# YifYang993/CR-NeRF-PyTorch

Measured on AMD Instinct MI355X. Metric: rays/sec (64+128 samples, 8-layer W=256 MLP), higher is better.
Workload: dtype f32

## Files before the change

cr-nerf-pytorch_amd/csrc/mlp_core.h:

```cpp
#pragma once
#include <hip/hip_runtime.h>
#include "layout.h"

namespace crnerf {

typedef float f32x16 __attribute__((ext_vector_type(16)));
typedef float f32x4 __attribute__((ext_vector_type(4)));
typedef __attribute__((address_space(3))) char lds_char;
typedef __attribute__((address_space(3))) float lds_float;
typedef __attribute__((address_space(3))) uint32_t lds_uint;
typedef const __attribute__((address_space(1))) char gbl_char;

constexpr int RING_SLOTS = 6;
static_assert(RING_SLOTS >= 5, "ring too shallow for the read-ahead protocol");

constexpr int LDS_CONST0 = 0;
constexpr int LDS_CONST1 = CONST_BYTES;
constexpr int LDS_RING = 2 * CONST_BYTES;
constexpr int LDS_SCRATCH = LDS_RING + RING_SLOTS * STAGE_BYTES;

enum { T_PROLOGUE = 0, T_MMA, T_EPILOGUE, T_SIGMA, T_COMPOSITE, T_RAYLEVEL, T_TOTAL, T_X0, T_X1, T_X2, T_X3, T_X4, T_X5, T_X6, T_X7, T_REAL, T_COUNT };
#ifdef CRNERF_TIMING
static __device__ unsigned long long crnerf_timing[T_COUNT];
struct PhaseTimer {
  unsigned long long last, acc[T_COUNT], real0;
  bool on;
  __device__ __forceinline__ void start(bool on_) {
    on = on_;
    for (int i = 0; i < T_COUNT; ++i) acc[i] = 0;
    real0 = __builtin_amdgcn_s_memrealtime();
    last = __builtin_readcyclecounter();
  }
  __device__ __forceinline__ void tick(int phase) {
    __builtin_amdgcn_sched_barrier(0);
    const unsigned long long t = __builtin_readcyclecounter();
    __builtin_amdgcn_sched_barrier(0);
    acc[phase] += t - last;
    acc[T_TOTAL] += t - last;
    last = t;
  }
  __device__ __forceinline__ void flush() {
    acc[T_REAL] = __builtin_amdgcn_s_memrealtime() - real0;
    if (on)
      for (int i = 0; i < T_COUNT; ++i) crnerf_timing[i] = acc[i];
  }
};
#else
struct PhaseTimer {
  __device__ __forceinline__ void start(bool) {}
  __device__ __forceinline__ void tick(int) {}
  __device__ __forceinline__ void flush() {}
};
#endif

__device__ __forceinline__ void glds16(uint32_t lds_addr, const char* base, uint32_t voff, int imm) {
#ifdef CRNERF_GLDS_SALU_COPY
  uint64_t b;
  asm volatile("s_mov_b32 m0, %1\n\ts_mov_b64 %0, %3\n\tglobal_load_lds_dwordx4 %2, %0 offset:%4"
               : "=&s"(b) : "s"(lds_addr), "v"(voff), "s"(base), "n"(imm) : "memory");
#else
  asm volatile("s_mov_b32 m0, %0\n\ts_nop 0\n\tglobal_load_lds_dwordx4 %1, %2 offset:%3" ::"s"(lds_addr), "v"(voff), "s"(base), "n"(imm)
               : "memory");
#endif
}
__device__ __forceinline__ void glds16_more(const char* base, uint32_t voff, int imm) {
#ifdef CRNERF_GLDS_SALU_COPY
  uint64_t b;
  asm volatile("s_mov_b64 %0, %2\n\tglobal_load_lds_dwordx4 %1, %0 offset:%3" : "=&s"(b) : "v"(voff), "s"(base), "n"(imm) : "memory");
#else
  asm volatile("global_load_lds_dwordx4 %0, %1 offset:%2" ::"v"(voff), "s"(base), "n"(imm) : "memory");
#endif
}

template <int NT>
__device__ __forceinline__ void init_acc(f32x16 (&acc)[NT], const lds_float* bias, int h) {
#pragma unroll
  for (int t = 0; t < NT; ++t) {
#pragma unroll
    for (int q = 0; q < 4; ++q) {
      const f32x4 b = *(const __attribute__((address_space(3))) f32x4*)(bias + 32 * t + 8 * q + 4 * h);
      acc[t][4 * q + 0] = b[0];
      acc[t][4 * q + 1] = b[1];
      acc[t][4 * q + 2] = b[2];
      acc[t][4 * q + 3] = b[3];
    }
  }
}

template <int NT, int NDST>
__device__ __forceinline__ void store_act(const f32x16 (&acc)[NT], f32x16 (&act)[NDST], float floor_) {
#pragma unroll
  for (int t = 0; t < NT; ++t)
#pragma unroll
    for (int r = 0; r < 16; ++r) act[t][r] = fmaxf(acc[t][r], floor_);
}

__device__ __forceinline__ float softplus_ref(float x) {
  return x > 20.0f ? x : log1pf(expf(x));
}
__device__ __forceinline__ float sigmoid_ref(float x) { return 1.0f / (1.0f + expf(-x)); }

__device__ __forceinline__ void load_consts(lds_char* lds, const char* packed0, const char* packed1) {
  const int tid = threadIdx.x;
  for (int i = tid; i < CONST_BYTES / 16; i += blockDim.x) {
    const f32x4 a = *(const f32x4*)(packed0 + i * 16);
    const f32x4 b = *(const f32x4*)(packed1 + i * 16);
    *(__attribute__((address_space(3))) f32x4*)(lds + LDS_CONST0 + i * 16) = a;
    *(__attribute__((address_space(3))) f32x4*)(lds + LDS_CONST1 + i * 16) = b;
  }
  __syncthreads();
}

}
```

cr-nerf-pytorch_amd/csrc/mlp_core16.h:

```cpp
#pragma once
#include <hip/hip_runtime.h>
#include "layout.h"
#include "sincos_pow2.h"
#include "mlp_core.h"

namespace crnerf {

#define CRNERF_MFMA16(a, b, c) __builtin_amdgcn_mfma_f32_16x16x4f32((a), (b), (c), 0, 0, 0)

constexpr int V16_WAVES = 8;
constexpr int V16_PIECES = STAGE_FRAGS / V16_WAVES;
constexpr int V16_AHEAD = 4;

constexpr int U_XYZ = XYZ_PAD / 16;
constexpr int U_HID = W_HIDDEN / 16;
constexpr int U_DIR = DIR_PAD / 16;
constexpr int U_HALF = 128 / 16;

constexpr int TRUNK_STAGES = OFF_FIN / STAGE_FRAGS;
static_assert(OFF_FIN % STAGE_FRAGS == 0, "the trunk must be whole stages");
template <bool TRUNK0>
struct WeightPipe16T {
  static constexpr bool trunk0 = TRUNK0;
  lds_char* lds;
  const char* base[2];
  const char* pf_ptr;
  int pf_left, pf_pass, passes0, passes;
  int stages_per_pass = STAGES_PER_PASS;
  uint32_t pf_slot, rd_slot, rd_addr, lane16, wave2k, lds_ring;
  int stagger;

  __device__ __forceinline__ void issue_piece(int i) {
    const uint32_t dst = lds_ring + pf_slot * STAGE_BYTES;
    if (i == 0) glds16(dst, pf_ptr, lane16, 0);
    else glds16(dst, pf_ptr, lane16, FRAG_BYTES);
    if (i == V16_PIECES - 1) {
      pf_slot = (pf_slot + 1 == RING_SLOTS) ? 0u : pf_slot + 1;
      pf_ptr += STAGE_BYTES;
      if (--pf_left == 0) {
        pf_left = stages_per_pass;
        pf_pass = (pf_pass + 1 == passes) ? 0 : pf_pass + 1;
        pf_ptr = (pf_pass < passes0) ? base[0] : base[1];
        if (TRUNK0 && pf_pass < passes0) pf_left = TRUNK_STAGES;
      }
    }
  }

  __device__ __forceinline__ void start(lds_char* lds_, const char* stream0, const char* stream1, int passes0_, int passes_,
                                        int lane, int wave) {
    static_assert(V16_PIECES == 2, "issue_piece hard-codes the two instruction offsets");
    lds = lds_;
    lane16 = (uint32_t)lane * 16u;
    wave2k = (uint32_t)wave * (V16_PIECES * FRAG_BYTES);
    lds_ring = (uint32_t)(uintptr_t)lds_ + LDS_RING + wave2k;
    stagger = (wave >> 2) & 1;
    base[0] = stream0 + wave2k;
    base[1] = stream1 + wave2k;
    passes0 = passes0_;
    passes = passes_;
    pf_pass = 0;
    pf_left = (TRUNK0 && passes0 > 0) ? TRUNK_STAGES : stages_per_pass;
    pf_ptr = (passes0 > 0) ? base[0] : base[1];
    pf_slot = 0;
    rd_slot = 0;
    rd_addr = LDS_RING + lane16;
#pragma unroll
    for (int s = 0; s < RING_SLOTS - 1; ++s)
#pragma unroll
      for (int i = 0; i < V16_PIECES; ++i) issue_piece(i);
    asm volatile("s_waitcnt vmcnt(%0)" ::"n"(V16_PIECES * (RING_SLOTS - 3)) : "memory");
    __builtin_amdgcn_s_barrier();
  }

  __device__ __forceinline__ uint32_t next_addr() const {
    const uint32_t n = (rd_slot + 1 == RING_SLOTS) ? 0u : rd_slot + 1;
    return LDS_RING + n * STAGE_BYTES + lane16;
  }

  __device__ __forceinline__ void advance() {
    asm volatile("s_waitcnt vmcnt(%0)" ::"n"(V16_PIECES * (RING_SLOTS - 4)) : "memory");
    __builtin_amdgcn_s_barrier();
    rd_slot = (rd_slot + 1 == RING_SLOTS) ? 0u : rd_slot + 1;
    rd_addr = LDS_RING + rd_slot * STAGE_BYTES + lane16;
  }

  __device__ __forceinline__ f32x4 read_slot(int s) const {
    const uint32_t a = (s < STAGE_FRAGS) ? rd_addr + s * FRAG_BYTES : next_addr() + (s - STAGE_FRAGS) * FRAG_BYTES;
    return *(const __attribute__((address_space(3))) f32x4*)(lds + a);
  }

  __device__ __forceinline__ void prime(f32x4 (&q)[V16_AHEAD]) const {
#pragma unroll
    for (int i = 0; i < V16_AHEAD; ++i) q[i] = read_slot(i);
  }
};
typedef WeightPipe16T<false> WeightPipe16;

template <int NT>
__device__ __forceinline__ void init_acc16(f32x4 (&acc)[NT], const lds_float* bias, int g) {
#pragma unroll
  for (int T = 0; T < NT; ++T) acc[T] = *(const __attribute__((address_space(3))) f32x4*)(bias + 16 * T + 4 * g);
}

struct NoDeferred {
  static constexpr int pieces = 0;
  __device__ __forceinline__ void piece(int) const {}
};
template <class SAVE, int ND>
struct DeferredActs {
  static constexpr int pieces = ND;
  const SAVE& save;
  float* row;
  const f32x4 (&a)[16];
  __device__ __forceinline__ void piece(int T) const { save.piece(row, T, a[T]); }
};

template <int NT, int NGA, int NGB, int NA, int NB, class DEF = NoDeferred, class PIPE>
__device__ __forceinline__ void mma_layer16(PIPE& p, const f32x4 (&srcA)[NA], const f32x4 (&srcB)[NB], f32x4 (&acc)[NT],
                                            f32x4 (&q)[V16_AHEAD], const DEF& def = DEF()) {
  static_assert(NGA <= NA && NGB <= NB, "source too small");
  constexpr int NF = (NGA + NGB) * NT;
  static_assert(NF % STAGE_FRAGS == 0 && NT % 2 == 0, "layer must be whole stages");
  constexpr int STEPS = NF / 2;
  constexpr int STRIDE = DEF::pieces > 0 ? (STEPS / DEF::pieces >= 4 ? 4 : (STEPS / DEF::pieces >= 2 ? 2 : 1)) : 1;
  static_assert(DEF::pieces == 0 || STRIDE * DEF::pieces <= STEPS, "not enough steps to carry the deferred stores");
#pragma unroll
  for (int u = 0; u < NGA + NGB; ++u) {
#pragma unroll
    for (int T = 0; T < NT; T += 2) {
      const int f = u * NT + T;
      const int s = f % STAGE_FRAGS;
      if (s % 4 == 0 && ((s >> 2) & 1) == p.stagger) p.issue_piece(s >> 3);
      const f32x4 a0 = q[f % V16_AHEAD], a1 = q[(f + 1) % V16_AHEAD];
      q[f % V16_AHEAD] = p.read_slot(s + V16_AHEAD);
      q[(f + 1) % V16_AHEAD] = p.read_slot(s + 1 + V16_AHEAD);
#pragma unroll
      for (int r = 0; r < 4; ++r) {
        const float b = (u < NGA) ? srcA[u < NGA ? u : 0][r] : srcB[u < NGA ? 0 : u - NGA][r];
        acc[T] = CRNERF_MFMA16(a0[r], b, acc[T]);
        acc[T + 1] = CRNERF_MFMA16(a1[r], b, acc[T + 1]);
      }
      if (s == STAGE_FRAGS - 2) p.advance();
      if (DEF::pieces > 0) {
        const int step = f / 2;
        if (step % STRIDE == 0 && step / STRIDE < DEF::pieces) def.piece(step / STRIDE);
      }
    }
  }
}

template <int NT, bool RELU, int NDST>
__device__ __forceinline__ void store_act16(const f32x4 (&acc)[NT], f32x4 (&act)[NDST]) {
#pragma unroll
  for (int T = 0; T < NT; ++T)
#pragma unroll
    for (int r = 0; r < 4; ++r) act[T][r] = RELU ? fmaxf(acc[T][r], 0.0f) : acc[T][r];
}

struct NoSave {
  template <int NT>
  __device__ __forceinline__ void operator()(int, const f32x4 (&)[NT]) const {}
  template <int NT>
  __device__ __forceinline__ float* begin(int, const f32x4 (&)[NT]) const { return nullptr; }
  __device__ __forceinline__ void piece(float*, int, const f32x4&) const {}
};

struct DirRegs {
  f32x4 v[2];
  __device__ __forceinline__ void get(f32x4 (&o)[2]) const { o[0] = v[0]; o[1] = v[1]; }
};
struct DirLds {
  const lds_float* p;
  __device__ __forceinline__ void get(f32x4 (&o)[2]) const {
    o[0] = *(const __attribute__((address_space(3))) f32x4*)(p);
    o[1] = *(const __attribute__((address_space(3))) f32x4*)(p + 4);
  }
};

template <class DIR, class SAVE = NoSave, class PIPE>
__device__ __forceinline__ void mlp_tile16(PIPE& p, int model, const f32x4 (&pe)[6], const DIR& dir,
                                           f32x4 (&feat)[4], float& sigma, int g, f32x4 (&q)[V16_AHEAD], PhaseTimer& tm,
                                           const SAVE& save = SAVE()) {
  const lds_float* C = (const lds_float*)(p.lds + (model ? LDS_CONST1 : LDS_CONST0));
  f32x4 act[16], acc[16];
  tm.tick(T_PROLOGUE);

  typedef DeferredActs<SAVE, 16> Def16;
  init_acc16<16>(acc, C + C_BIAS, g);
  mma_layer16<16, U_XYZ, 0>(p, pe, pe, acc, q);
  tm.tick(T_MMA);
  store_act16<16, true>(acc, act);
  float* row = save.begin(0, act);
#pragma unroll 1
  for (int l = 1; l < 4; ++l) {
    init_acc16<16>(acc, C + C_BIAS + l * W_HIDDEN, g);
    tm.tick(T_EPILOGUE);
    mma_layer16<16, U_HID, 0>(p, act, act, acc, q, Def16{save, row, act});
    tm.tick(T_MMA);
    store_act16<16, true>(acc, act);
    row = save.begin(l, act);
  }
  init_acc16<16>(acc, C + C_BIAS + 4 * W_HIDDEN, g);
  tm.tick(T_EPILOGUE);
  mma_layer16<16, U_XYZ, U_HID>(p, pe, act, acc, q, Def16{save, row, act});
  tm.tick(T_MMA);
  store_act16<16, true>(acc, act);
  row = save.begin(4, act);
#pragma unroll 1
  for (int l = 5; l < 8; ++l) {
    init_acc16<16>(acc, C + C_BIAS + l * W_HIDDEN, g);
    tm.tick(T_EPILOGUE);
    mma_layer16<16, U_HID, 0>(p, act, act, acc, q, Def16{save, row, act});
    tm.tick(T_MMA);
    store_act16<16, true>(acc, act);
    row = save.begin(l, act);
  }
  {
    float s0 = 0.0f, s1 = 0.0f;
#pragma unroll
    for (int T = 0; T < 16; T += 2) {
      const f32x4 w0 = *(const __attribute__((address_space(3))) f32x4*)(C + C_WSIG + 16 * T + 4 * g);
      const f32x4 w1 = *(const __attribute__((address_space(3))) f32x4*)(C + C_WSIG + 16 * (T + 1) + 4 * g);
#pragma unroll
      for (int r = 0; r < 4; ++r) {
        s0 = fmaf(w0[r], act[T][r], s0);
        s1 = fmaf(w1[r], act[T + 1][r], s1);
      }
    }
    float s = s0 + s1;
    s += __shfl_xor(s, 16);
    s += __shfl_xor(s, 32);
    sigma = softplus_ref(s + C[C_BSIG]);
  }
  tm.tick(T_SIGMA);
  if (PIPE::trunk0 && model == 0) {
#pragma unroll
    for (int T = 0; T < 4; ++T) feat[T] = f32x4{0, 0, 0, 0};
    return;
  }
  init_acc16<16>(acc, C + C_BFIN, g);
  mma_layer16<16, U_HID, 0>(p, act, act, acc, q, Def16{save, row, act});
  tm.tick(T_MMA);
  store_act16<16, false>(acc, act);
  row = save.begin(8, act);
  {
    f32x4 acc8[8], dv[2];
    dir.get(dv);
    init_acc16<8>(acc8, C + C_BDIR, g);
    tm.tick(T_EPILOGUE);
    mma_layer16<8, U_HID, U_DIR>(p, act, dv, acc8, q, Def16{save, row, act});
    tm.tick(T_MMA);
    store_act16<8, true>(acc8, act);
    row = save.begin(9, act);
  }
  {
    f32x4 acc4[4];
    init_acc16<4>(acc4, C + C_BRGB, g);
    tm.tick(T_EPILOGUE);
    mma_layer16<4, U_HALF, 0>(p, act, act, acc4, q, DeferredActs<SAVE, 8>{save, row, act});
    tm.tick(T_MMA);
#pragma unroll
    for (int T = 0; T < 4; ++T)
#pragma unroll
      for (int r = 0; r < 4; ++r) feat[T][r] = sigmoid_ref(acc4[T][r]);
  }
  tm.tick(T_EPILOGUE);
}

template <int F, int NV>
__device__ __forceinline__ void posenc_regs16(float x, float y, float z, int g, f32x4 (&out)[NV]) {
  const Rev2Pi rx = to_rev2pi(x), ry = to_rev2pi(y), rz = to_rev2pi(z);
#pragma unroll
  for (int v = 0; v < NV; ++v)
#pragma unroll
    for (int pr = 0; pr < 2; ++pr) {
      const int a_lo = 8 * v + pr;
      const int a = a_lo + 2 * g;
      float e0, e1;
      if (a_lo + 6 < 3 * F) {
        const int f = a / 3, d = a - 3 * f;
        const Rev2Pi val = {d == 0 ? rx.p : (d == 1 ? ry.p : rz.p), d == 0 ? rx.e : (d == 1 ? ry.e : rz.e)};
        float s, c;
        sincos_rev2pi(val, f, s, c);
        e0 = s; e1 = c;
      } else {
        const bool trig = a < 3 * F;
        const int ac = trig ? a : 0;
        const int f = ac / 3, d = ac - 3 * f;
        const Rev2Pi val = {d == 0 ? rx.p : (d == 1 ? ry.p : rz.p), d == 0 ? rx.e : (d == 1 ? ry.e : rz.e)};
        float s, c;
        sincos_rev2pi(val, f, s, c);
        e0 = trig ? s : (a == 3 * F ? x : (a == 3 * F + 1 ? z : 0.0f));
        e1 = trig ? c : (a == 3 * F ? y : 0.0f);
      }
      out[v][2 * pr + 0] = e0;
      out[v][2 * pr + 1] = e1;
    }
}

}
```

cr-nerf-pytorch_amd/csrc/render_fused16.hip:

```cpp
#include <hip/hip_runtime.h>
#include "kernels.h"
#include "mlp_core16.h"
#include "mlp_train16.h"
#include "pair_ops.h"
#include "ray_ops.h"

namespace crnerf {

struct RenderParams16 {
  const char* packed0; const char* packed1;
  const float* rays; const float* view_dir; const float* z_coarse; const float* z_steps; const float* u; long u_stride;
  const float* noise_c; const float* noise_f; float noise_std; int use_disp;
  long R; int Nc, Ni, iters;
  unsigned int* sched;
  float* weights_c; float* feature_c; float* depth_c; float* weights_f; float* feature_f; float* depth_f; float* z_fine;
  unsigned long long rng_seed; long rng_ray_offset; int rng_flags; float perturb;
  float* z_coarse_out; float* noise_c_out; float* noise_f_out;
};

static __device__ unsigned int crnerf_sched16[SCHED_SLOTS][2];

struct NoHook {
  __device__ __forceinline__ NoSave saver(int, long, int, int, bool, int) const { return NoSave(); }
  __device__ __forceinline__ void raw(int, long, int, int, bool, int, const f32x4 (&)[4], float) const {}
};
struct TrainHook {
  float* acts[2];
  float* rawo[2];
  long R;
  __device__ __forceinline__ ActSaver saver(int pass, long r, int N, int n, bool ok, int g) const {
    return ActSaver{pass ? acts[1] : acts[0], R * N, r * N + n, ok, g};
  }
  __device__ __forceinline__ void raw(int pass, long r, int N, int n, bool ok, int g, const f32x4 (&feat)[4], float sigma) const {
    if (!ok) return;
    float* o = (pass ? rawo[1] : rawo[0]) + (r * N + n) * OUT_DIM;
#pragma unroll
    for (int T = 0; T < 4; ++T)
#pragma unroll
      for (int q = 0; q < 4; ++q) o[16 * T + 4 * g + q] = feat[T][q];
    if (g == 0) o[FEAT_DIM] = sigma;
  }
};

template <bool RNG, class HOOK, bool LEAN = false>
__device__ __forceinline__ void render_rays16_impl(const RenderParams16& a, const HOOK& hook) {
  extern __shared__ __attribute__((aligned(16))) char smem[];
  lds_char* lds = (lds_char*)smem;
  const int lane = threadIdx.x & 63;
  const int wave = __builtin_amdgcn_readfirstlane(threadIdx.x >> 6);
  const int p = lane & 15, g = lane >> 4;
  const int pair = wave >> 1, half = wave & 1;
  const int lane128 = half * 64 + lane;
  const int Nc = a.Nc, Ni = a.Ni, Nf = Nc + Ni;

  load_consts(lds, a.packed0, a.packed1);
  PairScratch scr;
  scr.bind(lds + LDS_SCRATCH + pair * PAIR_BYTES);
  lds_float* dirbuf = (lds_float*)(lds + LDS_SCRATCH + 4 * PAIR_BYTES) + wave * 32;

  const int steps_c = (Nc + 31) >> 5, steps_f = Ni > 0 ? (Nf + 31) >> 5 : 0;
  WeightPipe16T<LEAN> pipe;
  pipe.start(lds, a.packed0 + CONST_BYTES, a.packed1 + CONST_BYTES, steps_c, steps_c + steps_f, lane, wave);
  f32x4 q[V16_AHEAD];
  pipe.prime(q);
  PhaseTimer tm;
  tm.start(blockIdx.x == 0 && threadIdx.x == 0);

  __attribute__((address_space(3))) unsigned int* qslot =
      (__attribute__((address_space(3))) unsigned int*)(lds + LDS_SCRATCH + 4 * PAIR_BYTES + V16_WAVES * 32 * sizeof(float));
  const long quads = (a.R + 3) / 4;
  long quad = blockIdx.x;
#pragma unroll 1
  for (int it = 0; a.sched ? quad < quads : it < a.iters; ++it) {
    unsigned int nxt = 0;
    if (a.sched && threadIdx.x == 0) nxt = gridDim.x + atomicAdd(a.sched, 1u);
    const long rr = quad * 4 + pair;
    const bool ray_ok = rr < a.R;
    const long r = ray_ok ? rr : a.R - 1;
    const float* ray = a.rays + r * 8;
    const float ox = ray[0], oy = ray[1], oz = ray[2], dx = ray[3], dy = ray[4], dz = ray[5];
    const float near = ray[6], far = ray[7];
    {
      const float* vd = a.view_dir ? a.view_dir + r * 3 : ray + 3;
      f32x4 dv[2];
      posenc_regs16<DIR_FREQS, 2>(vd[0], vd[1], vd[2], g, dv);
      if (p == 0) {
        *(__attribute__((address_space(3))) f32x4*)(dirbuf + 8 * g) = dv[0];
        *(__attribute__((address_space(3))) f32x4*)(dirbuf + 8 * g + 4) = dv[1];
      }
    }
    const DirLds dirsrc{dirbuf + 8 * g};
    const RayRng rng{(uint32_t)(a.rng_seed & 0xffffffffu), (uint32_t)(a.rng_seed >> 32)};
    const long rng_ray = a.rng_ray_offset + r;
    for (int n = lane128; n < Nc; n += 128) {
      auto zlin = [&](int k) { return coarse_depth(near, far, a.z_steps ? a.z_steps[k] : linspace01(k, Nc), a.use_disp); };
      float zv;
      if (a.z_coarse) zv = a.z_coarse[r * Nc + n];
      else if (RNG && (a.rng_flags & 1)) {
        const float z0 = zlin(n);
        const float lower = n == 0 ? z0 : 0.5f * (zlin(n - 1) + z0);
        const float upper = n == Nc - 1 ? z0 : 0.5f * (z0 + zlin(n + 1));
        zv = lower + (upper - lower) * (a.perturb * rng.uniform(RNG_STREAM_JITTER, rng_ray, n));
      } else zv = zlin(n);
      scr.zc[n] = zv;
      if (RNG && a.z_coarse_out && ray_ok) a.z_coarse_out[r * Nc + n] = zv;
    }
    wg_barrier();

    const int npass = Ni > 0 ? 2 : 1;
#pragma unroll 1
    for (int pass = 0; pass < npass; ++pass) {
      const int N = pass ? Nf : Nc;
      const lds_float* zsrc = pass ? scr.zs : scr.zc;
      const float* noise_row = pass ? (a.noise_f ? a.noise_f + r * Nf : nullptr) : (a.noise_c ? a.noise_c + r * Nc : nullptr);
      float* weights_row = LEAN ? nullptr : (pass ? a.weights_f + r * Nf : a.weights_c + r * Nc);
      const bool compose = !LEAN || pass;
      double carry = 1.0;
      f32x4 facc[4];
#pragma unroll
      for (int T = 0; T < 4; ++T) facc[T] = f32x4{0, 0, 0, 0};
      float dacc = 0.0f;
      const int steps = (N + 31) >> 5;
#pragma unroll 1
      for (int k = 0; k < steps; ++k) {
        const int n = 32 * k + 16 * half + p;
        const bool valid = n < N;
        const int nc = valid ? n : N - 1;
        const float zn = zsrc[nc];
        const float znext = zsrc[nc + 1 < N ? nc + 1 : N - 1];
        const float x = ox + dx * zn, y = oy + dy * zn, z = oz + dz * zn;
        f32x4 pe[6], feat[4];
        posenc_regs16<XYZ_FREQS, 6>(x, y, z, g, pe);
        float sigma;
        mlp_tile16(pipe, pass, pe, dirsrc, feat, sigma, g, q, tm, hook.saver(pass, r, N, n, valid && ray_ok, g));
        hook.raw(pass, r, N, n, valid && ray_ok, g, feat, sigma);
        float noise = (noise_row && valid) ? noise_row[n] * a.noise_std : 0.0f;
        if (RNG && (a.rng_flags & 4) && valid) {
          const float draw = rng.normal(pass ? RNG_STREAM_NOISE_FINE : RNG_STREAM_NOISE_COARSE, rng_ray, n);
          noise = draw * a.noise_std;
          float* no = pass ? a.noise_f_out : a.noise_c_out;
          if (no && ray_ok && g == 0) no[r * N + n] = draw;
        }
        const float delta = (n == N - 1) ? 1e2f : znext - zn;
        const float alpha = valid ? 1.0f - expf(-delta * fmaxf(sigma + noise, 0.0f)) : 0.0f;
        double incl = (double)(1.0f - alpha);
#pragma unroll
        for (int d = 1; d < 16; d <<= 1) {
          const double o = shfl_up_f64(incl, d, 16);
          if (p >= d) incl *= o;
        }
        double excl = shfl_up_f64(incl, 1, 16);
        if (p == 0) excl = 1.0;
        const double tot = shfl_f64(incl, 15, 16);
        if (lane == 0) scr.xprod[half] = tot;
        wg_barrier();
        const double other = scr.xprod[half ^ 1];
        const double prod_a = half ? other : tot, prod_b = half ? tot : other;
        const float Tr = (float)(half ? carry * prod_a * excl : carry * excl);
        carry = carry * prod_a * prod_b;
        const float w = alpha * Tr;
        if (compose) {
#pragma unroll
          for (int T = 0; T < 4; ++T)
#pragma unroll
            for (int rr2 = 0; rr2 < 4; ++rr2) facc[T][rr2] += w * feat[T][rr2];
          dacc += w * zn;
        }
        if (valid && g == 0) {
          if (!LEAN && ray_ok) weights_row[n] = w;
          if (pass == 0) scr.wc[n] = w;
        }
        tm.tick(T_COMPOSITE);
      }
      {
#pragma unroll
        for (int d = 8; d >= 1; d >>= 1) if (compose) {
#pragma unroll
          for (int T = 0; T < 4; ++T)
#pragma unroll
            for (int rr2 = 0; rr2 < 4; ++rr2) facc[T][rr2] += __shfl_xor(facc[T][rr2], d);
          dacc += __shfl_xor(dacc, d);
        }
        if (compose && half == 1 && p == 0) {
#pragma unroll
          for (int T = 0; T < 4; ++T) *(__attribute__((address_space(3))) f32x4*)(scr.xfeat + 16 * T + 4 * g) = facc[T];
          if (g == 0) scr.xfeat[64] = dacc;
        }
      }
      wg_barrier();
      if (compose && half == 0 && p == 0 && ray_ok) {
        float* frow = (pass ? a.feature_f : a.feature_c) + r * FEAT_DIM;
#pragma unroll
        for (int T = 0; T < 4; ++T) {
          const f32x4 o = *(const __attribute__((address_space(3))) f32x4*)(scr.xfeat + 16 * T + 4 * g);
          *(f32x4*)(frow + 16 * T + 4 * g) = facc[T] + o;
        }
        if (g == 0) (pass ? a.depth_f : a.depth_c)[r] = dacc + scr.xfeat[64];
      }
      if (pass == 0 && Ni > 0) {
        sample_pdf_pair(scr, Nc, Ni, a.u ? a.u + r * a.u_stride : nullptr, lane, lane128, (RNG && (a.rng_flags & 2)) ? &rng : nullptr, rng_ray);
        wg_barrier();
        merge_sort_pair(scr, Nc, Ni, lane128);
        wg_barrier();
        if (a.z_fine && ray_ok)
          for (int n = lane128; n < Nf; n += 128) a.z_fine[r * Nf + n] = scr.zs[n];
      }
      tm.tick(T_RAYLEVEL);
    }
    if (a.sched && threadIdx.x == 0) *qslot = nxt;
    wg_barrier();
    quad = a.sched ? (long)__builtin_amdgcn_readfirstlane((int)*qslot) : quad + gridDim.x;
  }
  if (a.sched && threadIdx.x == 0 && atomicAdd(a.sched + 1, 1u) == gridDim.x - 1) {
    atomicExch(a.sched, 0u);
    atomicExch(a.sched + 1, 0u);
  }
  tm.flush();
  asm volatile("s_waitcnt vmcnt(0)" ::: "memory");
}

__global__ __launch_bounds__(512, 2) void render_rays16_kernel(RenderParams16 a) { render_rays16_impl<false>(a, NoHook{}); }
__global__ __launch_bounds__(512, 2) void render_rays16_rng_kernel(RenderParams16 a) { render_rays16_impl<true>(a, NoHook{}); }
__global__ __launch_bounds__(512, 2) void render_rays16_lean_kernel(RenderParams16 a) { render_rays16_impl<false, NoHook, true>(a, NoHook{}); }

__global__ __launch_bounds__(512, 2) void render_rays_train16_kernel(RenderParams16 a, TrainHook h) { render_rays16_impl<false>(a, h); }
__global__ __launch_bounds__(512, 2) void render_rays_train16_rng_kernel(RenderParams16 a, TrainHook h) { render_rays16_impl<true>(a, h); }

int launch_render_rays16(const RenderArgs& a, hipStream_t stream) {
  if (a.R <= 0) return 0;
  if (a.Nc < 2 || a.Nc > MAX_NC) return set_error(-2, "render_rays: N_samples must be in [2, 256] for the fused kernel");
  if (a.Ni < 0 || a.Ni > MAX_NI) return set_error(-2, "render_rays: N_importance must be in [0, 256] for the fused kernel");
  if (a.Ni > 0 && a.Nc < 3) return set_error(-2, "render_rays: hierarchical sampling needs N_samples >= 3");
  if (a.Ni > 0 && !a.packed_fine) return set_error(-3, "render_rays: N_importance > 0 but no fine model");
  RenderParams16 k;
  k.packed0 = (const char*)a.packed_coarse;
  k.packed1 = (const char*)(a.packed_fine ? a.packed_fine : a.packed_coarse);
  k.rays = a.rays; k.view_dir = a.view_dir; k.z_coarse = a.z_coarse; k.z_steps = a.z_steps; k.u = a.u; k.u_stride = a.u_stride;
  k.noise_c = a.noise_coarse; k.noise_f = a.noise_fine; k.noise_std = a.noise_std; k.use_disp = a.use_disp;
  k.R = a.R; k.Nc = a.Nc; k.Ni = a.Ni;
  k.weights_c = a.weights_coarse; k.feature_c = a.feature_coarse; k.depth_c = a.depth_coarse;
  k.weights_f = a.weights_fine; k.feature_f = a.feature_fine; k.depth_f = a.depth_fine; k.z_fine = a.z_fine;
  k.rng_seed = a.rng_seed; k.rng_ray_offset = a.rng_ray_offset; k.rng_flags = a.rng_flags; k.perturb = a.perturb;
  k.z_coarse_out = a.z_coarse_out; k.noise_c_out = a.noise_coarse_out; k.noise_f_out = a.noise_fine_out;
  const long quads = (a.R + 3) / 4;
  const int cus = num_cus();
  const int grid = (int)(quads < cus ? quads : cus);
  k.iters = (int)((quads + grid - 1) / grid);
  k.sched = k.iters > 1 ? sched_slot((const void*)crnerf_sched16) : nullptr;
  const size_t shmem = LDS_SCRATCH + 4 * PAIR_BYTES + V16_WAVES * 32 * sizeof(float) + 16;
  if (a.lean) {
    if (a.Ni < 1) return set_error(-2, "render_rays_lean: N_importance must be in [1, 256] (the coarse pass alone has nothing lean to return)");
    if (a.train_acts_coarse || a.rng_flags || a.z_coarse_out) return set_error(-3, "render_rays_lean: inference only, random draws come as tensors");
    if (int rc = ensure_dynamic_lds((const void*)render_rays16_lean_kernel, shmem, "render_rays16_lean_kernel")) return rc;
    hipLaunchKernelGGL(render_rays16_lean_kernel, dim3(grid), dim3(512), shmem, stream, k);
    return check_launch("render_rays16_lean_kernel");
  }
  if (a.train_acts_coarse) {
    if (a.Ni > 0 && (!a.train_acts_fine || !a.train_raw_fine)) return set_error(-1, "render_rays_train: fine buffers are NULL");
    if (!a.train_raw_coarse) return set_error(-1, "render_rays_train: raw_coarse is NULL");
    TrainHook h{{(float*)a.train_acts_coarse, (float*)a.train_acts_fine}, {a.train_raw_coarse, a.train_raw_fine}, a.R};
    if (int rc = zero_acts_range(a.train_acts_coarse, a.R * a.Nc, stream)) return rc;
    if (a.Ni > 0)
      if (int rc = zero_acts_range(a.train_acts_fine, a.R * (a.Nc + a.Ni), stream)) return rc;
    const bool rngk = a.rng_flags != 0 || a.z_coarse_out;
    const void* fn = rngk ? (const void*)render_rays_train16_rng_kernel : (const void*)render_rays_train16_kernel;
    if (int rc = ensure_dynamic_lds(fn, shmem, "render_rays_train16_kernel")) return rc;
    if (rngk) hipLaunchKernelGGL(render_rays_train16_rng_kernel, dim3(grid), dim3(512), shmem, stream, k, h);
    else hipLaunchKernelGGL(render_rays_train16_kernel, dim3(grid), dim3(512), shmem, stream, k, h);
    return check_launch("render_rays_train16_kernel");
  }
  const bool rngk = a.rng_flags != 0 || a.z_coarse_out;
  const void* fn = rngk ? (const void*)render_rays16_rng_kernel : (const void*)render_rays16_kernel;
  if (int rc = ensure_dynamic_lds(fn, shmem, "render_rays16_kernel")) return rc;
  if (rngk) hipLaunchKernelGGL(render_rays16_rng_kernel, dim3(grid), dim3(512), shmem, stream, k);
  else hipLaunchKernelGGL(render_rays16_kernel, dim3(grid), dim3(512), shmem, stream, k);
  return check_launch("render_rays16_kernel");
}

#ifdef CRNERF_TIMING
extern "C" int crnerf_debug_read_timing16(unsigned long long* host_out) {
  return (int)hipMemcpyFromSymbol(host_out, HIP_SYMBOL(crnerf_timing), sizeof(unsigned long long) * T_COUNT);
}
#endif

}
```

Before: 442,300.

## Deepen weight ring to seven slots and barrier every other stage

Adds a seventh LDS ring slot for streamed weight stages. The waitcnt-plus-workgroup-barrier handshake now runs only on every second stage advance, which halves the number of barriers in the MMA loop. To make room in LDS for the extra slot, the per-wave direction buffer and the queue slot are moved into unused words of the pair scratch exchange block. The trade-offs are fewer stages prefetched ahead relative to ring depth and a tight LDS budget, checked by static asserts.

Result: no change. 442,300 (median of 5 runs) (-0.0%).

```diff
diff --git a/cr-nerf-pytorch_amd/csrc/mlp_core.h b/cr-nerf-pytorch_amd/csrc/mlp_core.h
--- a/cr-nerf-pytorch_amd/csrc/mlp_core.h
+++ b/cr-nerf-pytorch_amd/csrc/mlp_core.h
@@ -11,13 +11,16 @@
 typedef __attribute__((address_space(3))) uint32_t lds_uint;
 typedef const __attribute__((address_space(1))) char gbl_char;
 
-constexpr int RING_SLOTS = 6;
-static_assert(RING_SLOTS >= 5, "ring too shallow for the read-ahead protocol");
+constexpr int RING_SLOTS = 7;
+constexpr int RING_VM_STAGES = 2;
+static_assert(RING_SLOTS == 2 + 3 + RING_VM_STAGES, "free + readable + in-flight slots: ring depth, issue distance and vmcnt window go together (see above)");
 
 constexpr int LDS_CONST0 = 0;
 constexpr int LDS_CONST1 = CONST_BYTES;
 constexpr int LDS_RING = 2 * CONST_BYTES;
 constexpr int LDS_SCRATCH = LDS_RING + RING_SLOTS * STAGE_BYTES;
+constexpr int LDS_WORKGROUP_MAX = 160 * 1024;
+static_assert(LDS_SCRATCH <= LDS_WORKGROUP_MAX, "consts + ring exceed a workgroup's LDS");
 
 enum { T_PROLOGUE = 0, T_MMA, T_EPILOGUE, T_SIGMA, T_COMPOSITE, T_RAYLEVEL, T_TOTAL, T_X0, T_X1, T_X2, T_X3, T_X4, T_X5, T_X6, T_X7, T_REAL, T_COUNT };
 #ifdef CRNERF_TIMING
diff --git a/cr-nerf-pytorch_amd/csrc/mlp_core16.h b/cr-nerf-pytorch_amd/csrc/mlp_core16.h
--- a/cr-nerf-pytorch_amd/csrc/mlp_core16.h
+++ b/cr-nerf-pytorch_amd/csrc/mlp_core16.h
@@ -28,6 +28,7 @@
   int pf_left, pf_pass, passes0, passes;
   int stages_per_pass = STAGES_PER_PASS;
   uint32_t pf_slot, rd_slot, rd_addr, lane16, wave2k, lds_ring;
+  uint32_t meet;
   int stagger;
 
   __device__ __forceinline__ void issue_piece(int i) {
@@ -64,11 +65,12 @@
     pf_slot = 0;
     rd_slot = 0;
     rd_addr = LDS_RING + lane16;
-#pragma unroll
-    for (int s = 0; s < RING_SLOTS - 1; ++s)
+    meet = 0;
+#pragma unroll
+    for (int s = 0; s < RING_SLOTS - 2; ++s)
 #pragma unroll
       for (int i = 0; i < V16_PIECES; ++i) issue_piece(i);
-    asm volatile("s_waitcnt vmcnt(%0)" ::"n"(V16_PIECES * (RING_SLOTS - 3)) : "memory");
+    asm volatile("s_waitcnt vmcnt(%0)" ::"n"(V16_PIECES * RING_VM_STAGES) : "memory");
     __builtin_amdgcn_s_barrier();
   }
 
@@ -78,8 +80,11 @@
   }
 
   __device__ __forceinline__ void advance() {
-    asm volatile("s_waitcnt vmcnt(%0)" ::"n"(V16_PIECES * (RING_SLOTS - 4)) : "memory");
-    __builtin_amdgcn_s_barrier();
+    if (meet) {
+      asm volatile("s_waitcnt vmcnt(%0)" ::"n"(V16_PIECES * RING_VM_STAGES) : "memory");
+      __builtin_amdgcn_s_barrier();
+    }
+    meet ^= 1u;
     rd_slot = (rd_slot + 1 == RING_SLOTS) ? 0u : rd_slot + 1;
     rd_addr = LDS_RING + rd_slot * STAGE_BYTES + lane16;
   }
diff --git a/cr-nerf-pytorch_amd/csrc/render_fused16.hip b/cr-nerf-pytorch_amd/csrc/render_fused16.hip
--- a/cr-nerf-pytorch_amd/csrc/render_fused16.hip
+++ b/cr-nerf-pytorch_amd/csrc/render_fused16.hip
@@ -20,6 +20,14 @@
 
 static __device__ unsigned int crnerf_sched16[SCHED_SLOTS][2];
 
+constexpr int XCH_DIR = 68;
+constexpr int XCH_DIR3 = 100;
+constexpr int XCH_QSLOT = 108;
+constexpr int RENDER16_LDS = LDS_SCRATCH + 4 * PAIR_BYTES;
+static_assert(XCH_DIR > FEAT_DIM && XCH_DIR % 4 == 0 && XCH_DIR + 24 <= 96 && XCH_DIR3 >= 100 && XCH_DIR3 % 4 == 0 && XCH_QSLOT >= XCH_DIR3 + 8 && XCH_QSLOT < 128,
+              "the parked words overlap xfeat / xprod or leave the exchange block");
+static_assert(RENDER16_LDS <= LDS_WORKGROUP_MAX, "consts + ring + pair scratch exceed a workgroup's LDS");
+
 struct NoHook {
   __device__ __forceinline__ NoSave saver(int, long, int, int, bool, int) const { return NoSave(); }
   __device__ __forceinline__ void raw(int, long, int, int, bool, int, const f32x4 (&)[4], float) const {}
@@ -56,7 +64,7 @@
   load_consts(lds, a.packed0, a.packed1);
   PairScratch scr;
   scr.bind(lds + LDS_SCRATCH + pair * PAIR_BYTES);
-  lds_float* dirbuf = (lds_float*)(lds + LDS_SCRATCH + 4 * PAIR_BYTES) + wave * 32;
+  lds_float* dirbuf = scr.xfeat + (g < 3 ? XCH_DIR + 8 * g : XCH_DIR3);
 
   const int steps_c = (Nc + 31) >> 5, steps_f = Ni > 0 ? (Nf + 31) >> 5 : 0;
   WeightPipe16T<LEAN> pipe;
@@ -67,7 +75,7 @@
   tm.start(blockIdx.x == 0 && threadIdx.x == 0);
 
   __attribute__((address_space(3))) unsigned int* qslot =
-      (__attribute__((address_space(3))) unsigned int*)(lds + LDS_SCRATCH + 4 * PAIR_BYTES + V16_WAVES * 32 * sizeof(float));
+      (__attribute__((address_space(3))) unsigned int*)(lds + LDS_SCRATCH + (PAIR_FLOATS - 128 + XCH_QSLOT) * sizeof(float));
   const long quads = (a.R + 3) / 4;
   long quad = blockIdx.x;
 #pragma unroll 1
@@ -84,12 +92,12 @@
       const float* vd = a.view_dir ? a.view_dir + r * 3 : ray + 3;
       f32x4 dv[2];
       posenc_regs16<DIR_FREQS, 2>(vd[0], vd[1], vd[2], g, dv);
-      if (p == 0) {
-        *(__attribute__((address_space(3))) f32x4*)(dirbuf + 8 * g) = dv[0];
-        *(__attribute__((address_space(3))) f32x4*)(dirbuf + 8 * g + 4) = dv[1];
+      if (p == 0 && half == 0) {
+        *(__attribute__((address_space(3))) f32x4*)(dirbuf) = dv[0];
+        *(__attribute__((address_space(3))) f32x4*)(dirbuf + 4) = dv[1];
       }
     }
-    const DirLds dirsrc{dirbuf + 8 * g};
+    const DirLds dirsrc{dirbuf};
     const RayRng rng{(uint32_t)(a.rng_seed & 0xffffffffu), (uint32_t)(a.rng_seed >> 32)};
     const long rng_ray = a.rng_ray_offset + r;
     for (int n = lane128; n < Nc; n += 128) {
@@ -247,7 +255,7 @@
   const int grid = (int)(quads < cus ? quads : cus);
   k.iters = (int)((quads + grid - 1) / grid);
   k.sched = k.iters > 1 ? sched_slot((const void*)crnerf_sched16) : nullptr;
-  const size_t shmem = LDS_SCRATCH + 4 * PAIR_BYTES + V16_WAVES * 32 * sizeof(float) + 16;
+  const size_t shmem = RENDER16_LDS;
   if (a.lean) {
     if (a.Ni < 1) return set_error(-2, "render_rays_lean: N_importance must be in [1, 256] (the coarse pass alone has nothing lean to return)");
     if (a.train_acts_coarse || a.rng_flags || a.z_coarse_out) return set_error(-3, "render_rays_lean: inference only, random draws come as tensors");
```
